# cc-ai/MUNIT

Measured on AMD Instinct MI355X. Metric: images/sec (gen_update+dis_update) @256x256 bs=8, higher is better.
Workload: dtype f32; 1 GPU; config_256.yaml AdaINGen_double+MsImageDis dis_update+gen_update, 256x256, per-GPU batch 8, fp32; global_batch=8, parallelism=dp1, gen_state=1

## Files before the change

### include/munit_hip.h

```cpp
#ifndef MUNIT_HIP_H
#define MUNIT_HIP_H

#include <stddef.h>
#include <stdint.h>

#ifdef __cplusplus
extern "C" {
#endif

typedef void* munit_stream_t;

enum { MUNIT_OK = 0, MUNIT_ERR_ARG = -1, MUNIT_ERR_WORKSPACE = -2, MUNIT_ERR_LAUNCH = -3 };
enum { MUNIT_ACT_NONE = 0, MUNIT_ACT_RELU = 1, MUNIT_ACT_LRELU = 2, MUNIT_ACT_TANH = 3 };
enum { MUNIT_PAD_ZERO = 0, MUNIT_PAD_REFLECT = 1 };
enum { MUNIT_COMPUTE_F32 = 0, MUNIT_COMPUTE_BF16 = 1, MUNIT_COMPUTE_F32X3 = 2 };
enum { MUNIT_DTYPE_F32 = 0, MUNIT_DTYPE_BF16 = 1 };

int munit_version(void);
const char* munit_last_error(void);

typedef void* munit_comm_t;
int munit_comm_unique_id(void* id_out, size_t bytes);
int munit_comm_init(munit_comm_t* comm, int rank, int world, const void* unique_id);
int munit_comm_allreduce(munit_comm_t comm, float* buf, size_t count, munit_stream_t stream);
// ... 11 lines not shown
  float slope;
  int compute;
  int in_dtype, out_dtype;
} munit_conv_desc;

int munit_conv2d_out_hw(const munit_conv_desc* d, int* Ho, int* Wo);

size_t munit_conv2d_fwd_workspace_bytes(const munit_conv_desc* d);
int munit_conv2d_fwd(const munit_conv_desc* d, const void* x, const float* w, const float* bias,
                     void* y, void* ws, size_t ws_bytes, munit_stream_t stream);

size_t munit_conv2d_dgrad_workspace_bytes(const munit_conv_desc* d);
int munit_conv2d_dgrad(const munit_conv_desc* d, const void* dy, const float* w, const void* add,
                       void* dx, void* ws, size_t ws_bytes, munit_stream_t stream);

size_t munit_conv2d_wgrad_workspace_bytes(const munit_conv_desc* d);
int munit_conv2d_wgrad(const munit_conv_desc* d, const void* x, const void* dy, float* dw,
                       float* db, float beta, void* ws, size_t ws_bytes, munit_stream_t stream);

enum { MUNIT_PASS_FWD = 0, MUNIT_PASS_DGRAD = 1, MUNIT_PASS_WGRAD = 2 };
enum { MUNIT_PREP_NONE = 0, MUNIT_PREP_DGRAD = 1, MUNIT_PREP_SUBPIXEL = 2, MUNIT_PREP_CAST = 3,
       MUNIT_PREP_WINOGRAD = 4, MUNIT_PREP_WINOGRAD_DGRAD = 5, MUNIT_PREP_SUBPIXEL_WINOGRAD = 6,
       MUNIT_PREP_WINOGRAD_S2 = 7, MUNIT_PREP_WINOGRAD_S2_DGRAD = 8,
       MUNIT_PREP_SUBPIXEL_WINOGRAD_DGRAD = 9  };
typedef struct {
  const float* w;
  float* wp;
  int Cout, KH, KW, Cin;
  int kind;
  int ps;
  int bf16;
} munit_prep_item;
size_t munit_conv2d_prepared_weight_bytes(const munit_conv_desc* d, int pass);
int munit_conv2d_prep_item(const munit_conv_desc* d, int pass, const float* w, float* wp, munit_prep_item* out);
int munit_conv2d_prepare_weights(const munit_prep_item* item, munit_stream_t stream);
int munit_conv2d_prepare_weights_batch(const munit_prep_item* items_dev, int n, munit_stream_t stream);
int munit_conv2d_fwd_prepared(const munit_conv_desc* d, const void* x, const float* w, const void* wp,
                              const float* bias, void* y, void* ws, size_t ws_bytes, munit_stream_t stream);
int munit_conv2d_dgrad_prepared(const munit_conv_desc* d, const void* dy, const float* w, const void* wp,
                                const void* add, void* dx, void* ws, size_t ws_bytes, munit_stream_t stream);

size_t munit_linear_workspace_bytes(int B, int K, int N);
int munit_linear_fwd(const float* x, const float* w, const float* bias, float* y, int B, int K, int N, int act,
                     float slope, void* ws, size_t ws_bytes, munit_stream_t stream);
int munit_linear_bwd(const float* x, const float* w, const float* dy, float* dx, float* dw, float* db, int B, int K,
                     int N, float beta, void* ws, size_t ws_bytes, munit_stream_t stream);

// ... 189 lines not shown
```

### munit_amd/_lib.py

```python
import ctypes
import os
from ctypes import POINTER, Structure, c_char_p, c_double, c_float, c_int, c_size_t, c_void_p

_HERE = os.path.dirname(os.path.abspath(__file__))
LIB_PATH = os.environ.get("MUNIT_HIP_LIB") or os.path.join(_HERE, "libmunit_hip.so")

ACT = {"none": 0, "relu": 1, "lrelu": 2, "tanh": 3}
PAD = {"zero": 0, "reflect": 1}
COMPUTE = {"f32": 0, "bf16": 1, "f32x3": 2}
DTYPE = {"f32": 0, "bf16": 1}


class ConvDesc(Structure):
    _fields_ = [("B", c_int), ("H", c_int), ("W", c_int), ("Cin", c_int),
                ("Cout", c_int), ("KH", c_int), ("KW", c_int),
                ("stride", c_int), ("pad", c_int), ("pad_mode", c_int),
                ("upsample", c_int), ("act", c_int), ("slope", c_float), ("compute", c_int),
                ("in_dtype", c_int), ("out_dtype", c_int)]


class PrepItem(Structure):
    _fields_ = [("w", c_void_p), ("wp", c_void_p), ("Cout", c_int), ("KH", c_int), ("KW", c_int), ("Cin", c_int),
                ("kind", c_int), ("ps", c_int), ("bf16", c_int)]

# ... 117 lines not shown
    "munit_batchnorm_dp_workspace_bytes": (c_size_t, [c_int]),
    "munit_batchnorm_dp_stats_local": (c_int, [_P, ctypes.c_longlong, c_int, c_int, c_int, _P, c_size_t, _P, c_size_t, _P]),
    "munit_batchnorm_dp_fwd_apply": (c_int, [_P, _P, _P, _P, _P, _P, ctypes.c_longlong, c_int, c_int, _P, c_size_t, _P, _P,
                                             c_int, c_float, c_float, _P]),
    "munit_batchnorm_dp_bwd_local": (c_int, [_P, _P, _P, _P, _P, ctypes.c_longlong, c_int, c_int, c_int, c_int, _P, c_size_t,
                                             _P, c_size_t, _P]),
    "munit_batchnorm_dp_bwd_finish": (c_int, [_P, _P, _P, _P, _P, _P, _P, _P, _P, c_float, ctypes.c_longlong, c_int, c_int,
                                              c_int, c_int, _P, c_size_t, _P, c_size_t, _P]),
    "munit_maxpool2_fwd": (c_int, [_P, _P, _P, c_int, c_int, c_int, c_int, _P]),
    "munit_maxpool2_bwd": (c_int, [_P, _P, _P, c_int, c_int, c_int, c_int, _P]),
    "munit_avgpool16_fwd": (c_int, [_P, _P, c_int, c_int, c_int, c_int, _P]),
    "munit_avgpool16_bwd": (c_int, [_P, _P, c_int, c_int, c_int, c_int, _P]),
    "munit_gemm_f32": (c_int, [POINTER(GemmProblem), c_int, c_int, c_int, c_int, c_int, c_int, c_int, c_int, c_float,
                               c_float, _P]),
    "munit_fid_moments_workspace_bytes": (c_size_t, [c_int, c_int]),
    "munit_fid_moments": (c_int, [_P, c_int, c_int, _P, _P, _P, c_size_t, _P]),
    "munit_sqrt_newton_schulz_workspace_bytes": (c_size_t, [c_int, c_int]),
    "munit_sqrt_newton_schulz": (c_int, [_P, c_int, c_int, c_int, _P, _P, c_size_t, _P]),
    "munit_frechet_distance_workspace_bytes": (c_size_t, [c_int]),
    "munit_frechet_distance": (c_int, [_P, _P, _P, _P, c_int, c_int, _P, _P, c_size_t, _P]),
}

_lib = None


def load():
    global _lib
    if _lib is not None:
        return _lib
    if not os.path.exists(LIB_PATH):
        raise RuntimeError(
            "munit_amd: %s not found. Build it with `python -c 'import __graft_entry__ as g; g.build()'` "
            "(or `make -C munit_amd/csrc`). There is no CPU / PyTorch fallback." % LIB_PATH)
    lib = ctypes.CDLL(LIB_PATH)
    for name, (res, args) in SIGNATURES.items():
        try:
            fn = getattr(lib, name)
        except AttributeError as e:
            raise RuntimeError("munit_amd: %s does not export %s" % (LIB_PATH, name)) from e
        fn.restype = res
        fn.argtypes = args
    _lib = lib
    return lib


def check(rc, what=""):
    if rc != 0:
        msg = load().munit_last_error()
        raise RuntimeError("munit_hip %s failed (rc=%d): %s" % (what, rc, (msg or b"").decode()))
```

### munit_amd/csrc/common.h

```cpp
#pragma once
#include <hip/hip_runtime.h>
#include <cstdarg>
#include <cstdio>
#include <cstdlib>
#include "../../include/munit_hip.h"

typedef float f32x4 __attribute__((ext_vector_type(4)));
typedef float f32x16 __attribute__((ext_vector_type(16)));

typedef __bf16 bf16_t;
typedef __bf16 bf16v4 __attribute__((ext_vector_type(4)));
typedef __bf16 bf16v8 __attribute__((ext_vector_type(8)));

__device__ inline f32x4 ld4(const float* p) { return *reinterpret_cast<const f32x4*>(p); }
__device__ inline f32x4 ld4(const bf16_t* p) {
  const bf16v4 h = *reinterpret_cast<const bf16v4*>(p);
  return f32x4{(float)h[0], (float)h[1], (float)h[2], (float)h[3]};
}
__device__ inline void st4(float* p, f32x4 v) { *reinterpret_cast<f32x4*>(p) = v; }
__device__ inline void st4(bf16_t* p, f32x4 v) {
  *reinterpret_cast<bf16v4*>(p) = bf16v4{(bf16_t)v[0], (bf16_t)v[1], (bf16_t)v[2], (bf16_t)v[3]};
}
__device__ inline float ld1(const float* p) { return *p; }
__device__ inline float ld1(const bf16_t* p) { return (float)*p; }
// ... 28 lines not shown
#pragma unroll
  for (int off = 32; off > 0; off >>= 1) v += __shfl_xor(v, off, 64);
  return v;
}

__device__ inline float apply_act(float v, int act, float slope) {
  if (act == MUNIT_ACT_RELU) return v > 0.f ? v : 0.f;
  if (act == MUNIT_ACT_LRELU) return v > 0.f ? v : v * slope;
  if (act == MUNIT_ACT_TANH) return tanhf(v);
  return v;
}

__device__ inline int src_coord(int v, int Hu, int ups, int reflect) {
  const bool inside = v >= 0 && v < Hu;
  int r = v < 0 ? -v : v;
  r = r >= Hu ? 2 * Hu - 2 - r : r;
  r = reflect ? r : (inside ? v : -1);
  return r < 0 ? -1 : (r >> ups);
}

double munit_igemm_executed_flops(const munit_conv_desc* d, int pass);
const char* munit_igemm_kernel_name(const munit_conv_desc* d, int pass);

bool munit_small_fwd_supported(const munit_conv_desc* d);
bool munit_small_fwd_ok(const munit_conv_desc* d);
bool munit_small_wgrad_ok(const munit_conv_desc* d);
enum SmallFwdKernel { SMALL_FWD_PK, SMALL_FWD_MFMA, SMALL_FWD_PATCH };
SmallFwdKernel munit_small_fwd_kernel(int Cin);
bool munit_small_wgrad_pk();
size_t munit_small_fwd_workspace(const munit_conv_desc* d);
int munit_small_fwd(const munit_conv_desc* d, int Ho, int Wo, const void* x, const float* w, const float* bias,
                    float* y, void* ws, hipStream_t st);
size_t munit_small_wgrad_workspace(const munit_conv_desc* d, int Ho);
int munit_small_wgrad(const munit_conv_desc* d, int Ho, int Wo, const void* x, const float* dy, float* dw,
                      float* db, float beta, void* ws, hipStream_t st);
```

### munit_amd/csrc/conv_igemm.hip

```cpp
#include "common.h"
#include "wino.h"
#include <cstdlib>

namespace {

struct IgemmParams {
  const float* x;
  const float* w;
  const float* bias;
  void* y;
  int B, H, W, Cin;
  int Hu, Wu, ups;
  int Ho, Wo, Cout;
  int KH, KW, stride, pad, reflect;
  int Ktot;
  long long w_row;
  long long y_sb;
  long long y_sh;
  int y_sw;
  int M;
  int act;
  float slope;
  int ps;
  long long w_phase;
// ... 699 lines not shown
  const int dw = (int)(r % 3); r /= 3;
  const int dh = (int)(r % 3); r /= 3;
  const int co = (int)(r % it.Cout); r /= it.Cout;
  const int ph = (int)r;
  const int a = ph >> 1, b = ph & 1;
  const int h0 = a == 0 ? (dh == 0 ? 0 : dh == 1 ? 2 : 4) : (dh == 0 ? 0 : dh == 1 ? 1 : 3);
  const int hn = a == 0 ? (dh == 2 ? 1 : 2) : (dh == 0 ? 1 : 2);
  const int w0 = b == 0 ? (dw == 0 ? 0 : dw == 1 ? 2 : 4) : (dw == 0 ? 0 : dw == 1 ? 1 : 3);
  const int wn = b == 0 ? (dw == 2 ? 1 : 2) : (dw == 0 ? 1 : 2);
  float s = 0.f;
  for (int kh = h0; kh < h0 + hn; ++kh)
    for (int kw = w0; kw < w0 + wn; ++kw) s += it.w[(((long long)co * 5 + kh) * 5 + kw) * it.Cin + ci];
  if (it.bf16) reinterpret_cast<bf16_t*>(it.wp)[i] = (bf16_t)s;
  else it.wp[i] = s;
}

__host__ __device__ inline long long prep_elems(const PrepItem& it) {
  const long long cc = (long long)it.Cout * it.Cin;
  if (it.kind == MUNIT_PREP_SUBPIXEL) return it.bf16 ? (4 * 9 + 25) * cc : 4 * 9 * cc;
  if (it.kind == MUNIT_PREP_WINOGRAD || it.kind == MUNIT_PREP_WINOGRAD_DGRAD) return wino_image_elems(it.Cin, it.Cout);
  if (it.kind == MUNIT_PREP_SUBPIXEL_WINOGRAD_DGRAD) return cc * it.KH * it.KW + 4 * wino_image_elems(it.Cin, it.Cout);
  if (it.kind == MUNIT_PREP_SUBPIXEL_WINOGRAD || it.kind == MUNIT_PREP_WINOGRAD_S2 || it.kind == MUNIT_PREP_WINOGRAD_S2_DGRAD)
    return 4 * wino_image_elems(it.Cin, it.Cout);
  return cc * it.KH * it.KW;
}

__host__ __device__ inline long long prep_trips(const PrepItem& it) {
  const bool wino = it.kind == MUNIT_PREP_WINOGRAD || it.kind == MUNIT_PREP_WINOGRAD_DGRAD || it.kind == MUNIT_PREP_SUBPIXEL_WINOGRAD ||
                    it.kind == MUNIT_PREP_WINOGRAD_S2 || it.kind == MUNIT_PREP_WINOGRAD_S2_DGRAD;
  if (it.kind == MUNIT_PREP_SUBPIXEL_WINOGRAD_DGRAD) return (long long)it.Cout * it.Cin * (it.KH * it.KW + 4);
  return wino ? prep_elems(it) / 16 : prep_elems(it);
}
template <bool DEV>
__global__ void prep_weights_kernel(const PrepItem* __restrict__ items, PrepItem one) {
  const PrepItem it = DEV ? items[blockIdx.y] : one;
  const long long total = prep_trips(it);
  for (long long i = (long long)blockIdx.x * blockDim.x + threadIdx.x; i < total; i += (long long)gridDim.x * blockDim.x) {
    if (it.kind == MUNIT_PREP_SUBPIXEL) prep_subpixel_elem(it, i);
    else if (it.kind == MUNIT_PREP_WINOGRAD || it.kind == MUNIT_PREP_WINOGRAD_DGRAD)
      wino_weight_item(it.w, it.wp, it.Cout, it.Cin, it.kind == MUNIT_PREP_WINOGRAD_DGRAD, i);
    else if (it.kind == MUNIT_PREP_SUBPIXEL_WINOGRAD) wino_subpixel_weight_item(it.w, it.wp, it.Cout, it.Cin, i);
    else if (it.kind == MUNIT_PREP_WINOGRAD_S2) wino_s2_weight_item(it.w, it.wp, it.Cout, it.Cin, i);
    else if (it.kind == MUNIT_PREP_WINOGRAD_S2_DGRAD) wino_s2_dgrad_weight_item(it.w, it.wp, it.Cout, it.Cin, i);
    else if (it.kind == MUNIT_PREP_SUBPIXEL_WINOGRAD_DGRAD) {
      const long long nd = (long long)it.Cout * it.Cin * it.KH * it.KW;
      if (i < nd) prep_dgrad_elem(it, i);
      else wino_subpixel_dgrad_weight_item(it.w, it.wp + nd, it.Cout, it.Cin, i - nd);
    }
    else if (it.kind == MUNIT_PREP_CAST) prep_cast_elem(it, i);
    else prep_dgrad_elem(it, i);
  }
}

int launch_prep_one(const PrepItem& it, hipStream_t st) {
  const long long total = prep_trips(it);
  const int blocks = (int)std::min<long long>((total + 255) / 256, 4096);
  hipLaunchKernelGGL(prep_weights_kernel<false>, dim3(blocks), dim3(256), 0, st, nullptr, it);
  MUNIT_CHECK_LAUNCH("prep_weights");
  return MUNIT_OK;
}

template <typename T>
__global__ void fold_kernel(const T* __restrict__ g, const T* __restrict__ add,
                            T* __restrict__ dx, int B, int H, int W, int C, int ups, int pad,
                            int reflect, int Hq, int Wq) {
  const int C4 = C >> 2;
  const long long total = (long long)B * H * W * C4;
  const int Hu = H << ups, Wu = W << ups;
  for (long long i = (long long)blockIdx.x * blockDim.x + threadIdx.x; i < total;
       i += (long long)gridDim.x * blockDim.x) {
    long long r_ = i;
    int c4 = (int)(r_ % C4); r_ /= C4;
// ... 294 lines not shown
  q.ups = 0; q.Hu = d->H; q.Wu = d->W;
  q.Ho = d->H; q.Wo = d->W;
  q.KH = 3; q.KW = 3; q.pad = 1; q.reflect = 0;
  q.Ktot = 9 * d->Cin; q.w_row = q.Ktot;
  q.y_sw = 2 * d->Cout;
  q.y_sh = (long long)2 * Wo * d->Cout;
  q.M = d->B * d->H * d->W;
  q.ps = 2;
  q.w_phase = (long long)d->Cout * q.Ktot;
  q.y_phase_row = (long long)Wo * d->Cout;
  q.y_phase_col = d->Cout;
  return q;
}
void set_subpixel_frame(IgemmParams* p, const munit_conv_desc* d, int Ho, int Wo, int ring) {
  p->frame = ring;
  p->M = d->B * (2 * ring * Wo + 2 * ring * (Ho - 2 * ring));
}

bool wino_geometry_ok(const munit_conv_desc* d) {
  return d->compute == MUNIT_COMPUTE_F32 && d->in_dtype == MUNIT_DTYPE_F32 && d->out_dtype == MUNIT_DTYPE_F32 &&
         d->KH == 3 && d->KW == 3 && d->stride == 1 && d->pad == 1 && d->upsample == 0 && d->act != MUNIT_ACT_TANH;
}
bool wino_fwd_ok(const munit_conv_desc* d) { return wino_geometry_ok(d) && munit_wino_ok(d->B, d->H, d->W, d->Cin, d->Cout); }
long long wino_s2_min_blocks(bool dgrad) {
  static const char* const e = getenv("MUNIT_WINO_S2_MIN_BLOCKS");
  static const long long v = e ? atoll(e) : 0;
  return e ? v : dgrad ? 100 : 192;
}
bool wino_s2_fwd_ok(const munit_conv_desc* d) {
  return d->compute == MUNIT_COMPUTE_F32 && d->in_dtype == MUNIT_DTYPE_F32 && d->out_dtype == MUNIT_DTYPE_F32 && d->KH == 4 &&
         d->KW == 4 && d->stride == 2 && d->pad == 1 && d->upsample == 0 && d->act != MUNIT_ACT_TANH && d->H >= 4 && d->W >= 4 &&
         munit_wino_ok(d->B, d->H, d->W, d->Cin, d->Cout) && !MUNIT_ENV_FLAG("MUNIT_DEBUG_NO_WINOGRAD_S2") &&
         (long long)cdiv((long long)d->B * cdiv(d->H / 2, 3) * cdiv(d->W / 2, 3), 64) * (d->Cout / 64) >= wino_s2_min_blocks(false);
}
bool wino_s2_dgrad_ok(const munit_conv_desc* d) {
  if (!(d->compute == MUNIT_COMPUTE_F32 && d->in_dtype == MUNIT_DTYPE_F32 && d->out_dtype == MUNIT_DTYPE_F32 && d->KH == 4 &&
        d->KW == 4 && d->stride == 2 && d->pad == 1 && d->upsample == 0 && d->H >= 4 && d->W >= 4 && d->H % 2 == 0 && d->W % 2 == 0 &&
        d->Cout % 8 == 0 && d->Cin % 64 == 0 && !MUNIT_ENV_FLAG("MUNIT_DEBUG_NO_WINOGRAD_S2") && !MUNIT_ENV_FLAG("MUNIT_DEBUG_NO_WINOGRAD")))
    return false;
  const int Hd = d->H / 2, Wd = d->W / 2;
  if (d->pad_mode == MUNIT_PAD_REFLECT && (Hd % 3 == 0 || Wd % 3 == 0)) return false;
  if ((long long)d->B * d->H * d->W * std::max(d->Cin, d->Cout) >= (1ll << 29)) return false;
  return (long long)cdiv((long long)d->B * cdiv(Hd + 1, 3) * cdiv(Wd + 1, 3), 64) * (d->Cin / 64) * 4 >= wino_s2_min_blocks(true);
}
bool subpixel_wino_ok(const munit_conv_desc* d) {
  return d->compute == MUNIT_COMPUTE_F32 && d->in_dtype == MUNIT_DTYPE_F32 && d->out_dtype == MUNIT_DTYPE_F32 &&
         d->act != MUNIT_ACT_TANH && munit_wino_ok(d->B, d->H, d->W, d->Cin, d->Cout);
}

enum FwdRoute { FWD_SMALL, FWD_SUBPIXEL_WINO, FWD_SUBPIXEL, FWD_WINO, FWD_WINO_S2, FWD_CIN4, FWD_IGEMM };
struct FwdPlan {
  int rc;
  FwdRoute route;
  int Ho, Wo;
  munit_prep_item prep;
  Cin4Plan cin4;
  int ring;
  size_t img_bytes, ws_bytes;
};
FwdPlan plan_fwd(const munit_conv_desc* d) {
  FwdPlan pl{};
  if ((pl.rc = munit_conv2d_out_hw(d, &pl.Ho, &pl.Wo)) != MUNIT_OK) return pl;
  const int Ho = pl.Ho, Wo = pl.Wo, Ktot = d->KH * d->KW * d->Cin;
  const bool bf16 = d->in_dtype == MUNIT_DTYPE_BF16;
  int kind = bf16 ? MUNIT_PREP_CAST : MUNIT_PREP_NONE;
  if (munit_small_fwd_ok(d)) {
    pl.route = FWD_SMALL; kind = MUNIT_PREP_NONE;
  } else if (subpixel_ok(d)) {
    const bool wino = subpixel_wino_ok(d);
    pl.route = wino ? FWD_SUBPIXEL_WINO : FWD_SUBPIXEL; kind = wino ? MUNIT_PREP_SUBPIXEL_WINOGRAD : MUNIT_PREP_SUBPIXEL;
    pl.ring = wino ? 1 : 2;
  } else if (wino_fwd_ok(d)) {
    pl.route = FWD_WINO; kind = MUNIT_PREP_WINOGRAD;
  } else if (wino_s2_fwd_ok(d)) {
    pl.route = FWD_WINO_S2; kind = MUNIT_PREP_WINOGRAD_S2;
  } else {
    pl.route = cin4_fwd_ok(d) ? FWD_CIN4 : FWD_IGEMM;
  }
  pl.prep = munit_prep_item{nullptr, nullptr, d->Cout, d->KH, d->KW, d->Cin, kind, 1, pl.route != FWD_SMALL && bf16};
  pl.ws_bytes = pl.img_bytes = kind == MUNIT_PREP_NONE ? 0 : align_up((size_t)prep_elems(pl.prep) * (bf16 ? 2 : 4), 256);
  if (pl.route == FWD_SMALL) pl.ws_bytes = munit_small_fwd_workspace(d);
  if (pl.route == FWD_CIN4) pl.cin4 = plan_cin4((long long)d->B * d->H * d->W, d->Cout, d->KH * d->KW), pl.ws_bytes = pl.cin4.x4_bytes + pl.cin4.w4_bytes;
  if (bf16 || munit_small_fwd_supported(d)) return pl;
  if (pl.ring)
    pl.ws_bytes += std::max(splitk_bytes(d->B * (4 * Wo + 4 * (Ho - 4)), d->Cout, Ktot, 1), splitk_bytes(d->B * (2 * Wo + 2 * (Ho - 2)), d->Cout, Ktot, 1));
  if (pl.route == FWD_IGEMM) pl.ws_bytes += splitk_bytes(d->B * Ho * Wo, d->Cout, Ktot, 1);
  return pl;
}

enum WinoForm { WINO_FWD, WINO_FWD_S2, WINO_FWD_SUBPIXEL, WINO_DGRAD, WINO_DGRAD_S2, WINO_DGRAD_UP };
WinoParams wino_params(const munit_conv_desc* d, int Ho, int Wo, WinoForm f, const float* x, const float* u, const float* bias, float* y) {
  const bool fwd = f <= WINO_FWD_SUBPIXEL, refl = d->pad_mode == MUNIT_PAD_REFLECT;
  WinoParams q{};
  q.x = x; q.u = u; q.bias = bias; q.y = y;
  q.B = d->B; q.H = d->H; q.W = d->W;
  q.xc = fwd ? d->Cin : d->Cout; q.N = fwd ? d->Cout : d->Cin; q.K = q.xc;
  const int oh = fwd ? Ho : d->H, ow = fwd ? Wo : d->W;
  q.y_sw = q.N; q.y_sh = (long long)ow * q.N; q.y_sb = (long long)oh * ow * q.N;
// ... 46 lines not shown
  const FwdPlan pl = plan_fwd(d);
  int rc = pl.rc;
  if (rc) return rc;
  const int Ho = pl.Ho, Wo = pl.Wo;
  MUNIT_CHECK_ARG(x && w && y, "conv2d_fwd: null pointer");
  MUNIT_CHECK_ARG(pl.route != FWD_SMALL || d->out_dtype == MUNIT_DTYPE_F32, "conv2d_fwd: the 3-channel image head writes fp32");
  hipStream_t st = (hipStream_t)stream;
  if (pl.ws_bytes != 0 && (ws == nullptr || ws_bytes < pl.ws_bytes)) {
    munit_set_error("conv2d_fwd: workspace %zu < %zu", ws_bytes, pl.ws_bytes);
    return MUNIT_ERR_WORKSPACE;
  }
  if (pl.route == FWD_SMALL) return munit_small_fwd(d, Ho, Wo, x, w, bias, reinterpret_cast<float*>(y), ws, st);
  const float* wimg = w;
  if (pl.prep.kind != MUNIT_PREP_NONE) {
    wimg = reinterpret_cast<const float*>(wp);
    if (wimg == nullptr) {
      munit_prep_item it = pl.prep;
      it.w = w; it.wp = reinterpret_cast<float*>(ws);
      rc = launch_prep_one(it, st);
      if (rc) return rc;
      wimg = it.wp;
    }
  }
  if (pl.route == FWD_WINO || pl.route == FWD_WINO_S2 || pl.route == FWD_SUBPIXEL_WINO) {
    const WinoForm f = pl.route == FWD_WINO ? WINO_FWD : pl.route == FWD_WINO_S2 ? WINO_FWD_S2 : WINO_FWD_SUBPIXEL;
    rc = munit_wino_launch(wino_params(d, Ho, Wo, f, reinterpret_cast<const float*>(x), wimg, bias, reinterpret_cast<float*>(y)), st);
    if (rc || pl.route != FWD_SUBPIXEL_WINO) return rc;
  }
  IgemmParams p = fwd_params(d, Ho, Wo);
  p.x = reinterpret_cast<const float*>(x); p.w = wimg; p.bias = bias; p.y = y;
  if (pl.route == FWD_CIN4) {
    const long long npix = (long long)d->B * d->H * d->W;
    rc = build_cin4(pl.cin4, reinterpret_cast<const float*>(x), npix, w, d->Cout, d->KH * d->KW, ws, st);
    if (rc) return rc;
    p.x = reinterpret_cast<const float*>(ws);
    p.w = reinterpret_cast<const float*>(reinterpret_cast<const char*>(ws) + pl.cin4.x4_bytes);
    set_cin4(&p, pl.cin4);
    return launch_igemm<0>(p, 1, st);
  }
  if (pl.ring) {
    if (pl.route == FWD_SUBPIXEL) rc = launch_igemm<0>(subpixel_phase_params(p, d, Wo), 4, st);
    if (rc) return rc;
    set_subpixel_frame(&p, d, Ho, Wo, pl.ring);
    p.w = pl.prep.bf16 ? reinterpret_cast<const float*>(reinterpret_cast<const bf16_t*>(wimg) + (size_t)4 * 9 * d->Cout * d->Cin) : w;
  }
  return launch_igemm<0>(p, 1, st, ws ? reinterpret_cast<char*>(ws) + pl.img_bytes : nullptr, ws ? ws_bytes - pl.img_bytes : 0);
// ... 333 lines not shown
  if (pass == MUNIT_PASS_FWD) {
    it = plan_fwd(d).prep;
  } else {
    const DgradPlan pl = plan_dgrad(d);
    if (pl.rc) return pl.rc;
    it = pl.prep;
  }
  it.w = w; it.wp = wp;
  *out = it;
  return MUNIT_OK;
}

extern "C" size_t munit_conv2d_prepared_weight_bytes(const munit_conv_desc* d, int pass) {
  munit_prep_item it;
  if (munit_conv2d_prep_item(d, pass, nullptr, nullptr, &it) || it.kind == MUNIT_PREP_NONE) return 0;
  return (size_t)prep_elems(it) * (it.bf16 ? 2 : 4);
}

extern "C" int munit_conv2d_prepare_weights(const munit_prep_item* item, munit_stream_t stream) {
  MUNIT_CHECK_ARG(item && item->w && item->wp, "conv2d_prepare_weights: null pointer");
  const bool wino = item->kind == MUNIT_PREP_WINOGRAD || item->kind == MUNIT_PREP_WINOGRAD_DGRAD;
  const bool spw = item->kind == MUNIT_PREP_SUBPIXEL_WINOGRAD || item->kind == MUNIT_PREP_SUBPIXEL_WINOGRAD_DGRAD;
  const bool ws2 = item->kind == MUNIT_PREP_WINOGRAD_S2 || item->kind == MUNIT_PREP_WINOGRAD_S2_DGRAD;
  MUNIT_CHECK_ARG(!ws2 || (item->KH == 4 && item->KW == 4 && !item->bf16 &&
                           (item->kind == MUNIT_PREP_WINOGRAD_S2 ? item->Cin % 8 == 0 && item->Cout % 64 == 0
                                                                 : item->Cout % 8 == 0 && item->Cin % 64 == 0)),
                  "conv2d_prepare_weights: stride-2 Winograd image needs a 4x4 fp32 filter, K %% 8 == 0, N %% 64 == 0");
  MUNIT_CHECK_ARG(!spw || (item->KH == 5 && item->KW == 5 && !item->bf16 &&
                           (item->kind != MUNIT_PREP_SUBPIXEL_WINOGRAD_DGRAD ? item->Cin % 8 == 0 && item->Cout % 64 == 0
                                                                       : item->Cout % 8 == 0 && item->Cin % 64 == 0)),
                  "conv2d_prepare_weights: sub-pixel Winograd image needs a 5x5 fp32 filter, Cin %% 8 == 0, Cout %% 64 == 0");
  MUNIT_CHECK_ARG(item->kind == MUNIT_PREP_DGRAD || item->kind == MUNIT_PREP_SUBPIXEL || wino || spw || ws2 || (item->kind == MUNIT_PREP_CAST && item->bf16),
                  "conv2d_prepare_weights: bad kind %d", item->kind);
  MUNIT_CHECK_ARG(!wino || (item->KH == 3 && item->KW == 3 && !item->bf16 &&
                            (item->kind != MUNIT_PREP_WINOGRAD_DGRAD ? item->Cin % 8 == 0 && item->Cout % 64 == 0
                                                               : item->Cout % 8 == 0 && item->Cin % 64 == 0)),
                  "conv2d_prepare_weights: Winograd image needs a 3x3 fp32 filter, K %% 8 == 0, N %% 64 == 0");
  MUNIT_CHECK_ARG(item->ps >= 1 && item->KH % item->ps == 0 && item->KW % item->ps == 0, "conv2d_prepare_weights: bad phase count");
  MUNIT_CHECK_ARG(item->kind != MUNIT_PREP_SUBPIXEL || (item->KH == 5 && item->KW == 5), "conv2d_prepare_weights: sub-pixel needs 5x5");
  return launch_prep_one(*item, (hipStream_t)stream);
}

extern "C" int munit_conv2d_prepare_weights_batch(const munit_prep_item* items_dev, int n, munit_stream_t stream) {
  MUNIT_CHECK_ARG(items_dev != nullptr && n > 0 && n <= 65535, "conv2d_prepare_weights_batch: bad table (n=%d)", n);
  hipLaunchKernelGGL(prep_weights_kernel<true>, dim3(64, (unsigned)n), dim3(256), 0, (hipStream_t)stream, items_dev, PrepItem{});
  MUNIT_CHECK_LAUNCH("prep_weights_batch");
  return MUNIT_OK;
}

namespace {
const char* igemm_refusal(IgemmForm f) {
  switch (f) {
    case IG_REFUSED_BF16_CIN: return "refused: bf16 storage needs a multiple of 64 input channels";
    case IG_REFUSED_CIN4_FOLD: return "refused: 4-channel taps are not a folded backward-data form";
    case IG_REFUSED_BF16_FOLD: return "refused: bf16-storage folded backward-data exists for the LDS-patch form only";
// ... 16 lines not shown
    const FwdPlan fp = plan_fwd(d);
    if (fp.rc) return "invalid";
    const int Ho = fp.Ho, Wo = fp.Wo;
    IgemmParams p = fwd_params(d, Ho, Wo);
    const int bn = igemm_bn(p);
    switch (fp.route) {
      case FWD_SMALL: return y_bf16 ? "refused: the 3-channel image head writes fp32" : head[0][munit_small_fwd_kernel(d->Cin)][x_bf16];
      case FWD_SUBPIXEL_WINO: return "conv_wino_kernel<1, 0> x4 sub-pixel phases + conv_igemm_kernel frame";
      case FWD_SUBPIXEL: {
        const IgemmForm ph = igemm_form(subpixel_phase_params(p, d, Wo), 0);
        set_subpixel_frame(&p, d, Ho, Wo, fp.ring);
        const IgemmForm fr = igemm_form(p, 0);
        if (igemm_refusal(ph)) return igemm_refusal(ph);
        if (igemm_refusal(fr)) return igemm_refusal(fr);
        if (ph != fr) return "invalid";
        if (ph == IG_BF16S) return bn == 64 ? "conv_igemm_kernel<64, true, 0, 4> x4 sub-pixel phases + frame"
                                            : "conv_igemm_kernel<128, true, 0, 4> x4 sub-pixel phases + frame";
        if (ph == IG_CT1) return "conv_igemm_kernel<.., 0, 1> x4 sub-pixel phases + frame";
        if (ph == IG_CT2) return "conv_igemm_kernel<.., 0, 2> x4 sub-pixel phases + frame";
        return "conv_igemm_kernel x4 sub-pixel phases + frame";
      }
      case FWD_WINO: return refl ? "conv_wino_kernel<0, 0>" : "conv_wino_kernel<1, 0>";
      case FWD_WINO_S2: return refl ? "conv_wino_kernel<0, 1>" : "conv_wino_kernel<1, 1>";
      case FWD_CIN4: set_cin4(&p, fp.cin4); break;
      case FWD_IGEMM: break;
    }
    const IgemmForm f = igemm_form(p, 0);
    if (igemm_refusal(f)) return igemm_refusal(f);
    if (fp.route == FWD_CIN4) return y_bf16 ? "conv_igemm_kernel<.., 5> (3 input channels as 4-channel taps, bf16 y)"
                                            : "conv_igemm_kernel<.., 5> (3 input channels as 4-channel taps)";
    if (f == IG_BF16S) return bn == 64 ? "conv_igemm_kernel<64, true, 0, 4>" : "conv_igemm_kernel<128, true, 0, 4>";
    if (f == IG_CT1) return "conv_igemm_kernel<.., 0, 1>";
    if (f == IG_CT2) return "conv_igemm_kernel<.., 0, 2>";
    return "conv_igemm_kernel<fwd>";
  }
  const DgradPlan pl = plan_dgrad(d);
  if (pl.rc) return "invalid";
  if (x_bf16 && d->Cin % 4 != 0) return "refused: bf16 dx needs Cin % 4 == 0";
  switch (pl.route) {
    case DG_WINO_S2: return refl ? "conv_wino_kernel<0, 2>" : "conv_wino_kernel<1, 2>";
    case DG_WINO: return refl ? "conv_wino_kernel<2, 0>" : "conv_wino_kernel<1, 0>";
    case DG_SMALL: return x_bf16 ? "refused: the 3-channel data gradient is fp32" : head[1][munit_small_fwd_kernel(d->Cout)][y_bf16];
    case DG_FOLD_UPWINO: case DG_FOLD_BOXSUM: case DG_FOLD: {
      if (!dgrad_fold_dtypes_ok(d, pl)) return "refused: unsupported dtype combination";
      IgemmParams p = dgrad_fold_params(d, pl);
      const int bn = igemm_bn(p);
// ... 33 lines not shown
    return "conv_igemm_kernel<dgrad direct>";
  }
  const bool fold16 = x_bf16 && fold_vectorised(d);
  if (f == IG_BF16S) {
    if (fold16) return bn == 64 ? "conv_igemm_kernel<64, true, 1, 4> phases + fold_kernel<bf16_t>" : "conv_igemm_kernel<128, true, 1, 4> phases + fold_kernel<bf16_t>";
    return bn == 64 ? "conv_igemm_kernel<64, true, 1, 4> phases + fold_kernel" : "conv_igemm_kernel<128, true, 1, 4> phases + fold_kernel";
  }
  if (f == IG_CT1) return fold16 ? "conv_igemm_kernel<.., 1, 1> phases + fold_kernel<bf16_t>" : "conv_igemm_kernel<.., 1, 1> phases + fold_kernel";
  if (f == IG_CT2) return fold16 ? "conv_igemm_kernel<.., 1, 2> phases + fold_kernel<bf16_t>" : "conv_igemm_kernel<.., 1, 2> phases + fold_kernel";
  return fold16 ? "conv_igemm_kernel<.., 1, .> phases + fold_kernel<bf16_t>" : "conv_igemm_kernel<.., 1, .> phases + fold_kernel";
}

double munit_igemm_executed_flops(const munit_conv_desc* d, int pass) {
  int Ho, Wo;
  if (munit_conv2d_out_hw(d, &Ho, &Wo)) return 0.0;
  const double cc = 2.0 * d->Cin * d->Cout;
  if (pass == MUNIT_PASS_FWD) {
    const FwdPlan fp = plan_fwd(d);
    switch (fp.route) {
      case FWD_SUBPIXEL_WINO: return cc * d->B * ((double)(d->H / 2) * (d->W / 2) * 4 * 16 + (2.0 * Wo + 2.0 * (Ho - 2)) * 25);
      case FWD_SUBPIXEL: return cc * d->B * ((double)d->H * d->W * 4 * 9 + (4.0 * Wo + 4.0 * (Ho - 4)) * 25);
      case FWD_WINO: return cc * d->B * (d->H / 2) * (d->W / 2) * 16;
      case FWD_WINO_S2: return 4 * cc * d->B * cdiv(Ho, 3) * cdiv(Wo, 3) * 16;
      case FWD_CIN4: return 2.0 * d->Cout * d->B * Ho * Wo * fp.cin4.kpad;
      default: return cc * d->B * Ho * Wo * d->KH * d->KW;
    }
  }
  const DgradPlan pl = plan_dgrad(d);
  if (pl.rc) return 0.0;
  switch (pl.route) {
    case DG_WINO_S2: return 4 * cc * d->B * cdiv(d->H / 2 + 1, 3) * cdiv(d->W / 2 + 1, 3) * 16;
    case DG_WINO: return cc * d->B * (d->H / 2) * (d->W / 2) * 16;
    case DG_FOLD_UPWINO: return cc * d->B * ((double)((d->H - 4) / 2) * ((d->W - 4) / 2) * 4 * 16 + (4.0 * d->W + 4.0 * (d->H - 4)) * 25);
    case DG_FOLD_BOXSUM: return cc * d->B * ((double)(d->H - 4) * (d->W - 4) + 4.0 * d->W + 4.0 * (d->H - 4)) * d->KH * d->KW;
    case DG_FOLD: return cc * d->B * d->H * d->W * d->KH * d->KW;
    case DG_DIRECT: return cc * d->B * Ho * Wo * d->KH * d->KW;
    case DG_CIN4: return 2.0 * d->Cin * d->B * (double)(pl.Ho + pl.TH - 1) * (pl.Wo + pl.TW - 1) * pl.cin4.kpad;
    case DG_SMALL: case DG_CORR: return cc * d->B * (double)(pl.Ho + pl.TH - 1) * (pl.Wo + pl.TW - 1) * pl.TH * pl.TW * pl.ps * pl.ps;
  }
  return 0.0;
}

namespace {
munit_conv_desc linear_desc(int B, int K, int N, int act, float slope, int compute) {
  munit_conv_desc d{};
  d.B = B; d.H = 1; d.W = 1; d.Cin = K; d.Cout = N; d.KH = 1; d.KW = 1; d.stride = 1; d.pad = 0;
  d.pad_mode = MUNIT_PAD_ZERO; d.upsample = 0; d.act = act; d.slope = slope; d.compute = compute;
  return d;
}
// ... 32 lines not shown
```

### munit_amd/csrc/conv_small.hip

```cpp
#include "common.h"

namespace {

struct SmallParams {
  const void* x;
  const float* w;
  const float* bias;
  const float* dy;
  float* y;
  float* slab;
  int B, H, W, Cin, Ho, Wo;
  int pad, reflect, act;
  float slope;
  int tiles_x, tiles_y;
  int rows_per_unit, units_per_img;
};

__device__ inline int map_coord(int v, int n, int reflect) {
  if (v < 0) return reflect ? -v : -1;
  if (v >= n) return reflect ? 2 * n - 2 - v : -1;
  return v;
}

template <int CO, int K, typename XT>
// ... 382 lines not shown
}

__global__ void small_slab_reduce_kernel(const float* __restrict__ slab, float* __restrict__ dw,
                                         float* __restrict__ db, long long n_w, int co, long long rows,
                                         float beta) {
  const long long stride = n_w + co;
  for (long long i = (long long)blockIdx.x * blockDim.x + threadIdx.x; i < stride;
       i += (long long)gridDim.x * blockDim.x) {
    float s0 = 0.f, s1 = 0.f, s2 = 0.f, s3 = 0.f;
    long long r = 0;
    for (; r + 3 < rows; r += 4) {
      s0 += slab[r * stride + i];
      s1 += slab[(r + 1) * stride + i];
      s2 += slab[(r + 2) * stride + i];
      s3 += slab[(r + 3) * stride + i];
    }
    for (; r < rows; ++r) s0 += slab[r * stride + i];
    const float s = (s0 + s1) + (s2 + s3);
    if (i < n_w) dw[i] = (beta != 0.f ? beta * dw[i] : 0.f) + s;
    else if (db != nullptr) db[i - n_w] = (beta != 0.f ? beta * db[i - n_w] : 0.f) + s;
  }
}

}

namespace {
template <int CO, int K, typename XT>
__global__ __launch_bounds__(256) void conv_lanes_wgrad_pk_kernel(SmallParams p) {
  typedef float f32x2 __attribute__((ext_vector_type(2)));
  const int lane = threadIdx.x & 63;
  const int wv = __builtin_amdgcn_readfirstlane(threadIdx.x >> 6);
  const int G = p.Cin >> 6;
  const long long unit = (long long)blockIdx.x * 4 + wv;
  const long long per_band = (long long)K * G;
  const long long nunits = (long long)p.B * p.units_per_img * per_band;
  if (unit >= nunits) return;
  const int g = (int)(unit % G);
  const int kh = (int)((unit / G) % K);
  const long long band = unit / per_band;
  const int bi = (int)(band % p.units_per_img);
  const int b = (int)(band / p.units_per_img);
  const int rh = lane >> 5, cp = lane & 31;
  const int ci = g * 64 + 2 * cp;
  const bool want_b = g == 0 && kh == 0;

  f32x2 acc[CO][K];
// ... 158 lines not shown
```

### munit_amd/csrc/runtime.hip

```cpp
#include "common.h"
#include <cstring>

namespace {
thread_local char g_err[512] = "";
}

void munit_set_error(const char* fmt, ...) {
  va_list ap;
  va_start(ap, fmt);
  vsnprintf(g_err, sizeof(g_err), fmt, ap);
  va_end(ap);
}

extern "C" const char* munit_last_error(void) { return g_err; }
extern "C" int munit_version(void) { return 5; }

extern "C" int munit_stream_wait_stream(munit_stream_t waiter, munit_stream_t signaler) {
  constexpr int MAX_DEV = 16;
  static thread_local hipEvent_t ev[MAX_DEV] = {};
  int dev = 0;
  if (hipGetDevice(&dev) != hipSuccess || dev < 0 || dev >= MAX_DEV) {
    munit_set_error("stream_wait_stream: no current device");
    return MUNIT_ERR_ARG;
  }
  if (ev[dev] == nullptr && hipEventCreateWithFlags(&ev[dev], hipEventDisableTiming) != hipSuccess) {
    munit_set_error("stream_wait_stream: hipEventCreate failed");
    return MUNIT_ERR_LAUNCH;
  }
  hipEvent_t use = ev[dev];
  hipError_t e = hipEventRecord(use, (hipStream_t)signaler);
  if (e == hipSuccess) e = hipStreamWaitEvent((hipStream_t)waiter, use, 0);
  if (e != hipSuccess) {
    munit_set_error("stream_wait_stream: %s", hipGetErrorString(e));
    return MUNIT_ERR_LAUNCH;
  }
  return MUNIT_OK;
}
```

Before: 78.93 images/s.

## Add MFMA-based direct kernel for the first 7x7 Cin=3 convolution

Adds a dedicated forward kernel for the 7x7, stride-1, pad-3, three-channel input convolution that begins each encoder. It stages an input strip and a prepacked, zero-padded, swizzled weight image in shared memory and computes with 16x16x4 fp32 MFMA, replacing the generic cin4/igemm route for this layer. A new weight prep kind builds that image, the library version is bumped and checked from Python, and the Winograd-s2 block thresholds become compile-time and env overridable. The weight image pads the 21-wide kernel row to 24, so some arithmetic is wasted on zeros.

```diff
diff --git a/include/munit_hip.h b/include/munit_hip.h
--- a/include/munit_hip.h
+++ b/include/munit_hip.h
@@ -57,7 +57,8 @@
 enum { MUNIT_PREP_NONE = 0, MUNIT_PREP_DGRAD = 1, MUNIT_PREP_SUBPIXEL = 2, MUNIT_PREP_CAST = 3,
        MUNIT_PREP_WINOGRAD = 4, MUNIT_PREP_WINOGRAD_DGRAD = 5, MUNIT_PREP_SUBPIXEL_WINOGRAD = 6,
        MUNIT_PREP_WINOGRAD_S2 = 7, MUNIT_PREP_WINOGRAD_S2_DGRAD = 8,
-       MUNIT_PREP_SUBPIXEL_WINOGRAD_DGRAD = 9  };
+       MUNIT_PREP_SUBPIXEL_WINOGRAD_DGRAD = 9,
+       MUNIT_PREP_FIRST7 = 10 };
 typedef struct {
   const float* w;
   float* wp;
diff --git a/munit_amd/_lib.py b/munit_amd/_lib.py
--- a/munit_amd/_lib.py
+++ b/munit_amd/_lib.py
@@ -163,6 +163,7 @@
 }
 
 _lib = None
+VERSION = 6
 
 
 def load():
@@ -181,6 +182,9 @@
             raise RuntimeError("munit_amd: %s does not export %s" % (LIB_PATH, name)) from e
         fn.restype = res
         fn.argtypes = args
+    if lib.munit_version() != VERSION:
+        raise RuntimeError("munit_amd: %s is version %d, this package needs %d: rebuild it (`make -C munit_amd/csrc`)"
+                           % (LIB_PATH, lib.munit_version(), VERSION))
     _lib = lib
     return lib
 
diff --git a/munit_amd/csrc/common.h b/munit_amd/csrc/common.h
--- a/munit_amd/csrc/common.h
+++ b/munit_amd/csrc/common.h
@@ -74,6 +74,17 @@
 double munit_igemm_executed_flops(const munit_conv_desc* d, int pass);
 const char* munit_igemm_kernel_name(const munit_conv_desc* d, int pass);
 
+constexpr int F7_KROW = 24, F7_IMG = 7 * F7_KROW * 64;
+__host__ __device__ inline long long first7_image_elems(int Cout) { return (long long)(Cout / 64) * F7_IMG; }
+__device__ inline float first7_image_elem(const float* __restrict__ w, long long i) {
+  const int nb = (int)(i / F7_IMG), r = (int)(i - (long long)nb * F7_IMG);
+  const int kh = r / (F7_KROW * 64), kk = (r >> 6) % F7_KROW, n = (r & 63) ^ ((kk & 1) << 4);
+  return kk < 21 ? w[((long long)(nb * 64 + n) * 7 + kh) * 21 + kk] : 0.f;
+}
+bool munit_first7_fwd_ok(const munit_conv_desc* d);
+int munit_first7_fwd(const munit_conv_desc* d, int Ho, int Wo, const float* x, const float* wimg, const float* bias,
+                     float* y, hipStream_t st);
+
 bool munit_small_fwd_supported(const munit_conv_desc* d);
 bool munit_small_fwd_ok(const munit_conv_desc* d);
 bool munit_small_wgrad_ok(const munit_conv_desc* d);
diff --git a/munit_amd/csrc/conv_igemm.hip b/munit_amd/csrc/conv_igemm.hip
--- a/munit_amd/csrc/conv_igemm.hip
+++ b/munit_amd/csrc/conv_igemm.hip
@@ -745,6 +745,7 @@
   if (it.kind == MUNIT_PREP_SUBPIXEL_WINOGRAD_DGRAD) return cc * it.KH * it.KW + 4 * wino_image_elems(it.Cin, it.Cout);
   if (it.kind == MUNIT_PREP_SUBPIXEL_WINOGRAD || it.kind == MUNIT_PREP_WINOGRAD_S2 || it.kind == MUNIT_PREP_WINOGRAD_S2_DGRAD)
     return 4 * wino_image_elems(it.Cin, it.Cout);
+  if (it.kind == MUNIT_PREP_FIRST7) return first7_image_elems(it.Cout);
   return cc * it.KH * it.KW;
 }
 
@@ -771,6 +772,7 @@
       else wino_subpixel_dgrad_weight_item(it.w, it.wp + nd, it.Cout, it.Cin, i - nd);
     }
     else if (it.kind == MUNIT_PREP_CAST) prep_cast_elem(it, i);
+    else if (it.kind == MUNIT_PREP_FIRST7) it.wp[i] = first7_image_elem(it.w, i);
     else prep_dgrad_elem(it, i);
   }
 }
@@ -1111,10 +1113,19 @@
          d->KH == 3 && d->KW == 3 && d->stride == 1 && d->pad == 1 && d->upsample == 0 && d->act != MUNIT_ACT_TANH;
 }
 bool wino_fwd_ok(const munit_conv_desc* d) { return wino_geometry_ok(d) && munit_wino_ok(d->B, d->H, d->W, d->Cin, d->Cout); }
+#ifndef MUNIT_WINO_S2_MIN_FWD
+#define MUNIT_WINO_S2_MIN_FWD 192
+#endif
+#ifndef MUNIT_WINO_S2_MIN_DGRAD
+#define MUNIT_WINO_S2_MIN_DGRAD 100
+#endif
+constexpr long long WINO_S2_MIN_FWD = MUNIT_WINO_S2_MIN_FWD, WINO_S2_MIN_DGRAD = MUNIT_WINO_S2_MIN_DGRAD;
 long long wino_s2_min_blocks(bool dgrad) {
   static const char* const e = getenv("MUNIT_WINO_S2_MIN_BLOCKS");
-  static const long long v = e ? atoll(e) : 0;
-  return e ? v : dgrad ? 100 : 192;
+  static const char* const ed = getenv("MUNIT_WINO_S2_MIN_BLOCKS_DGRAD");
+  static const long long v = e ? atoll(e) : 0, vd = ed ? atoll(ed) : 0;
+  if (dgrad && ed) return vd;
+  return e ? v : dgrad ? WINO_S2_MIN_DGRAD : WINO_S2_MIN_FWD;
 }
 bool wino_s2_fwd_ok(const munit_conv_desc* d) {
   return d->compute == MUNIT_COMPUTE_F32 && d->in_dtype == MUNIT_DTYPE_F32 && d->out_dtype == MUNIT_DTYPE_F32 && d->KH == 4 &&
@@ -1137,7 +1148,7 @@
          d->act != MUNIT_ACT_TANH && munit_wino_ok(d->B, d->H, d->W, d->Cin, d->Cout);
 }
 
-enum FwdRoute { FWD_SMALL, FWD_SUBPIXEL_WINO, FWD_SUBPIXEL, FWD_WINO, FWD_WINO_S2, FWD_CIN4, FWD_IGEMM };
+enum FwdRoute { FWD_SMALL, FWD_SUBPIXEL_WINO, FWD_SUBPIXEL, FWD_WINO, FWD_WINO_S2, FWD_FIRST7, FWD_CIN4, FWD_IGEMM };
 struct FwdPlan {
   int rc;
   FwdRoute route;
@@ -1163,6 +1174,8 @@
     pl.route = FWD_WINO; kind = MUNIT_PREP_WINOGRAD;
   } else if (wino_s2_fwd_ok(d)) {
     pl.route = FWD_WINO_S2; kind = MUNIT_PREP_WINOGRAD_S2;
+  } else if (munit_first7_fwd_ok(d)) {
+    pl.route = FWD_FIRST7; kind = MUNIT_PREP_FIRST7;
   } else {
     pl.route = cin4_fwd_ok(d) ? FWD_CIN4 : FWD_IGEMM;
   }
@@ -1255,6 +1268,8 @@
       wimg = it.wp;
     }
   }
+  if (pl.route == FWD_FIRST7)
+    return munit_first7_fwd(d, Ho, Wo, reinterpret_cast<const float*>(x), wimg, bias, reinterpret_cast<float*>(y), st);
   if (pl.route == FWD_WINO || pl.route == FWD_WINO_S2 || pl.route == FWD_SUBPIXEL_WINO) {
     const WinoForm f = pl.route == FWD_WINO ? WINO_FWD : pl.route == FWD_WINO_S2 ? WINO_FWD_S2 : WINO_FWD_SUBPIXEL;
     rc = munit_wino_launch(wino_params(d, Ho, Wo, f, reinterpret_cast<const float*>(x), wimg, bias, reinterpret_cast<float*>(y)), st);
@@ -1634,6 +1649,9 @@
   const bool wino = item->kind == MUNIT_PREP_WINOGRAD || item->kind == MUNIT_PREP_WINOGRAD_DGRAD;
   const bool spw = item->kind == MUNIT_PREP_SUBPIXEL_WINOGRAD || item->kind == MUNIT_PREP_SUBPIXEL_WINOGRAD_DGRAD;
   const bool ws2 = item->kind == MUNIT_PREP_WINOGRAD_S2 || item->kind == MUNIT_PREP_WINOGRAD_S2_DGRAD;
+  const bool f7 = item->kind == MUNIT_PREP_FIRST7;
+  MUNIT_CHECK_ARG(!f7 || (item->KH == 7 && item->KW == 7 && item->Cin == 3 && item->Cout % 64 == 0 && !item->bf16),
+                  "conv2d_prepare_weights: the first-layer image needs a 7x7 fp32 filter, Cin == 3, Cout %% 64 == 0");
   MUNIT_CHECK_ARG(!ws2 || (item->KH == 4 && item->KW == 4 && !item->bf16 &&
                            (item->kind == MUNIT_PREP_WINOGRAD_S2 ? item->Cin % 8 == 0 && item->Cout % 64 == 0
                                                                  : item->Cout % 8 == 0 && item->Cin % 64 == 0)),
@@ -1642,7 +1660,7 @@
                            (item->kind != MUNIT_PREP_SUBPIXEL_WINOGRAD_DGRAD ? item->Cin % 8 == 0 && item->Cout % 64 == 0
                                                                        : item->Cout % 8 == 0 && item->Cin % 64 == 0)),
                   "conv2d_prepare_weights: sub-pixel Winograd image needs a 5x5 fp32 filter, Cin %% 8 == 0, Cout %% 64 == 0");
-  MUNIT_CHECK_ARG(item->kind == MUNIT_PREP_DGRAD || item->kind == MUNIT_PREP_SUBPIXEL || wino || spw || ws2 || (item->kind == MUNIT_PREP_CAST && item->bf16),
+  MUNIT_CHECK_ARG(item->kind == MUNIT_PREP_DGRAD || item->kind == MUNIT_PREP_SUBPIXEL || wino || spw || ws2 || f7 || (item->kind == MUNIT_PREP_CAST && item->bf16),
                   "conv2d_prepare_weights: bad kind %d", item->kind);
   MUNIT_CHECK_ARG(!wino || (item->KH == 3 && item->KW == 3 && !item->bf16 &&
                             (item->kind != MUNIT_PREP_WINOGRAD_DGRAD ? item->Cin % 8 == 0 && item->Cout % 64 == 0
@@ -1705,6 +1723,7 @@
       }
       case FWD_WINO: return refl ? "conv_wino_kernel<0, 0>" : "conv_wino_kernel<1, 0>";
       case FWD_WINO_S2: return refl ? "conv_wino_kernel<0, 1>" : "conv_wino_kernel<1, 1>";
+      case FWD_FIRST7: return "conv_first7_kernel";
       case FWD_CIN4: set_cin4(&p, fp.cin4); break;
       case FWD_IGEMM: break;
     }
@@ -1784,9 +1803,11 @@
       case FWD_SUBPIXEL: return cc * d->B * ((double)d->H * d->W * 4 * 9 + (4.0 * Wo + 4.0 * (Ho - 4)) * 25);
       case FWD_WINO: return cc * d->B * (d->H / 2) * (d->W / 2) * 16;
       case FWD_WINO_S2: return 4 * cc * d->B * cdiv(Ho, 3) * cdiv(Wo, 3) * 16;
+      case FWD_FIRST7: return 2.0 * d->Cout * d->B * Ho * Wo * 7 * F7_KROW;
       case FWD_CIN4: return 2.0 * d->Cout * d->B * Ho * Wo * fp.cin4.kpad;
-      default: return cc * d->B * Ho * Wo * d->KH * d->KW;
-    }
+      case FWD_SMALL: case FWD_IGEMM: return cc * d->B * Ho * Wo * d->KH * d->KW;
+    }
+    return 0.0;
   }
   const DgradPlan pl = plan_dgrad(d);
   if (pl.rc) return 0.0;
diff --git a/munit_amd/csrc/conv_small.hip b/munit_amd/csrc/conv_small.hip
--- a/munit_amd/csrc/conv_small.hip
+++ b/munit_amd/csrc/conv_small.hip
@@ -428,6 +428,138 @@
   }
 }
 
+constexpr int F7_TW = 64, F7_TH = 8, F7_ROWS = F7_TH + 6, F7_RS = 216;
+static_assert(3 * (F7_TW - 1) + 4 * 5 + 3 < F7_RS && 3 * (F7_TW + 6) <= F7_RS, "fragment reads stay inside a strip row");
+
+struct First7Params {
+  const float* x;
+  const float* img;
+  const float* bias;
+  float* y;
+  int B, H, W, Cout;
+  int reflect, act;
+  float slope;
+  int tiles_x, tiles_y;
+};
+
+__device__ inline int first7_coord(int v, int n, int reflect) {
+  if (v < -3 || v > n + 2) return -1;
+  return map_coord(v, n, reflect);
+}
+
+__global__ __launch_bounds__(256, 2) void conv_first7_kernel(First7Params p) {
+  __shared__ __attribute__((aligned(16))) float wl[F7_IMG];
+  __shared__ __attribute__((aligned(16))) float strip[F7_ROWS * F7_RS];
+  const int tid = threadIdx.x, lane = tid & 63;
+  const int wv = __builtin_amdgcn_readfirstlane(tid >> 6);
+  const int j = lane & 15, g = lane >> 4;
+  int bid = blockIdx.x;
+  const int tile_x = bid % p.tiles_x; bid /= p.tiles_x;
+  const int tile_y = bid % p.tiles_y;
+  const int b = bid / p.tiles_y;
+  const int nb = blockIdx.y;
+  const int ow0 = tile_x * F7_TW, oh0 = tile_y * F7_TH;
+
+  {
+    const f32x4* __restrict__ src = reinterpret_cast<const f32x4*>(p.img + (long long)nb * F7_IMG);
+    f32x4* dst = reinterpret_cast<f32x4*>(wl);
+    for (int i = tid; i < F7_IMG / 4; i += 256) dst[i] = src[i];
+    const float* __restrict__ xb = p.x + (long long)b * p.H * p.W * 3;
+    constexpr int N = F7_ROWS * F7_RS, PER = (N + 255) / 256;
+    float stage[PER];
+#pragma unroll
+    for (int it = 0; it < PER; ++it) {
+      const int e = tid + 256 * it;
+      const int r = e / F7_RS, f = e - r * F7_RS;
+      const int c = f / 3, ch = f - 3 * c;
+      const int ih = first7_coord(oh0 + r - 3, p.H, p.reflect);
+      const int iw = first7_coord(ow0 + c - 3, p.W, p.reflect);
+      stage[it] = (e < N && c < F7_TW + 6 && ih >= 0 && iw >= 0) ? xb[((long long)ih * p.W + iw) * 3 + ch] : 0.f;
+    }
+#pragma unroll
+    for (int it = 0; it < PER; ++it) {
+      const int e = tid + 256 * it;
+      if (e < N) strip[e] = stage[it];
+    }
+  }
+  __syncthreads();
+
+  int wo[4];
+#pragma unroll
+  for (int nt = 0; nt < 4; ++nt) wo[nt] = g * 64 + ((16 * nt + j) ^ ((g & 1) << 4));
+  f32x4 bias4[4];
+#pragma unroll
+  for (int nt = 0; nt < 4; ++nt)
+    bias4[nt] = p.bias != nullptr ? ld4(p.bias + nb * 64 + 16 * nt + 4 * g) : f32x4{0.f, 0.f, 0.f, 0.f};
+
+#pragma unroll 1
+  for (int rr = 0; rr < 2; ++rr) {
+    const int row = wv + 4 * rr;
+    const int oh = oh0 + row;
+    if (oh >= p.H) break;
+    f32x4 acc[2][4][4];
+#pragma unroll
+    for (int c = 0; c < 2; ++c)
+#pragma unroll
+      for (int mt = 0; mt < 4; ++mt)
+#pragma unroll
+        for (int nt = 0; nt < 4; ++nt) acc[c][mt][nt] = f32x4{0.f, 0.f, 0.f, 0.f};
+    const float* sb = strip + row * F7_RS + 6 * j + g;
+#pragma unroll
+    for (int kh = 0; kh < 7; ++kh) {
+#pragma unroll
+      for (int ks = 0; ks < 6; ++ks) {
+        float a[4], bv[4];
+#pragma unroll
+        for (int nt = 0; nt < 4; ++nt) a[nt] = wl[(kh * F7_KROW + 4 * ks) * 64 + wo[nt]];
+#pragma unroll
+        for (int mt = 0; mt < 4; ++mt) bv[mt] = sb[kh * F7_RS + 96 * (mt >> 1) + 3 * (mt & 1) + 4 * ks];
+#pragma unroll
+        for (int mt = 0; mt < 4; ++mt)
+#pragma unroll
+          for (int nt = 0; nt < 4; ++nt)
+            acc[ks & 1][mt][nt] = __builtin_amdgcn_mfma_f32_16x16x4f32(a[nt], bv[mt], acc[ks & 1][mt][nt], 0, 0, 0);
+      }
+    }
+    float* yrow = p.y + ((long long)b * p.H + oh) * p.W * p.Cout + nb * 64 + 4 * g;
+#pragma unroll
+    for (int mt = 0; mt < 4; ++mt) {
+      const int ow = ow0 + 32 * (mt >> 1) + 2 * j + (mt & 1);
+      if (ow < p.W) {
+        float* yo = yrow + (long long)ow * p.Cout;
+#pragma unroll
+        for (int nt = 0; nt < 4; ++nt) {
+          f32x4 v = (acc[0][mt][nt] + acc[1][mt][nt]) + bias4[nt];
+#pragma unroll
+          for (int r = 0; r < 4; ++r) v[r] = apply_act(v[r], p.act, p.slope);
+          st4(yo + 16 * nt, v);
+        }
+      }
+    }
+  }
+}
+
+}
+
+bool munit_first7_fwd_ok(const munit_conv_desc* d) {
+  return d->Cin == 3 && d->KH == 7 && d->KW == 7 && d->stride == 1 && d->pad == 3 && d->upsample == 0 &&
+         d->compute == MUNIT_COMPUTE_F32 && d->in_dtype == MUNIT_DTYPE_F32 && d->out_dtype == MUNIT_DTYPE_F32 &&
+         d->Cout % 64 == 0 && d->act != MUNIT_ACT_TANH && (d->pad_mode != MUNIT_PAD_REFLECT || (d->H >= 4 && d->W >= 4)) &&
+         (long long)d->B * cdiv(d->H, F7_TH) * cdiv(d->W, F7_TW) < (1ll << 31) && !MUNIT_ENV_FLAG("MUNIT_DEBUG_NO_FIRST7");
+}
+
+int munit_first7_fwd(const munit_conv_desc* d, int Ho, int Wo, const float* x, const float* wimg, const float* bias,
+                     float* y, hipStream_t st) {
+  MUNIT_CHECK_ARG(Ho == d->H && Wo == d->W && wimg != nullptr, "conv_first7: bad geometry or null weight image");
+  First7Params p{};
+  p.x = x; p.img = wimg; p.bias = bias; p.y = y;
+  p.B = d->B; p.H = d->H; p.W = d->W; p.Cout = d->Cout;
+  p.reflect = d->pad_mode == MUNIT_PAD_REFLECT; p.act = d->act; p.slope = d->slope;
+  p.tiles_x = cdiv(Wo, F7_TW); p.tiles_y = cdiv(Ho, F7_TH);
+  const dim3 grid((unsigned)((long long)d->B * p.tiles_x * p.tiles_y), (unsigned)(d->Cout / 64));
+  hipLaunchKernelGGL(conv_first7_kernel, grid, dim3(256), 0, st, p);
+  MUNIT_CHECK_LAUNCH("conv_first7");
+  return MUNIT_OK;
 }
 
 namespace {
diff --git a/munit_amd/csrc/runtime.hip b/munit_amd/csrc/runtime.hip
--- a/munit_amd/csrc/runtime.hip
+++ b/munit_amd/csrc/runtime.hip
@@ -13,7 +13,7 @@
 }
 
 extern "C" const char* munit_last_error(void) { return g_err; }
-extern "C" int munit_version(void) { return 5; }
+extern "C" int munit_version(void) { return 6; }
 
 extern "C" int munit_stream_wait_stream(munit_stream_t waiter, munit_stream_t signaler) {
   constexpr int MAX_DEV = 16;
```

Result: no change. 79.49 images/s, median of 6 (+0.7%).
